# NeuroDiffGym/neurodiffeq

Hardware: AMD Instinct MI355X
Metric: collocation-points/sec (residual+bwd), 2D Laplace 65k pts, 1/2/4/8 GPU (higher is better)
Workload: dtype f32; 1 GPU; C2: Solver2D 2D Laplace, DirichletBVP2D, FCNN(2-32-32-1, tanh), Generator2D 256x256 = 65536 noisy-grid points per GPU per step, Adam(1e-3), run_train_epoch() with n_batches_train=1, n_batches_valid=0; points_per_gpu=65536, global_batch=65536, parallelism=dp1 (shard-by-batch, one all-reduce of [P+1] fp32 per step), allreduce=none (single process), inputs=pre-sampled in the reference's RNG order, resident in HBM

## Files before the change

### neurodiffeq_amd/_build.py

```python
import os

from . import _hipcc

HERE = os.path.dirname(os.path.abspath(__file__))
CSRC = os.path.join(HERE, "csrc")
LIB = os.path.join(HERE, "libndq.so")
SOURCES = [os.path.join(CSRC, "ndq_api.hip")]
HEADERS = [os.path.join(CSRC, h) for h in ("ndq_mlp.h", "ndq_tail.h", "ndq_launch.h", "ndq_wide.h", "ndq_deep.h", "ndq_sample.h", "ndq_oneshot.h")] + \
    [os.path.join(HERE, "..", "include", "ndq.h"), os.path.join(HERE, "_hipcc.py")]
LIB64 = os.path.join(HERE, "libndq64.so")
SOURCES64 = [os.path.join(CSRC, "ndq_api64.hip")]
FLAGS = []
_EXTRA = os.environ.get("NDQ_LIB_FLAGS", "").split()
if _EXTRA:
    import hashlib
    LIB = os.path.join(HERE, "libndq_" + hashlib.sha1(" ".join(_EXTRA).encode()).hexdigest()[:8] + ".so")
    FLAGS = FLAGS + _EXTRA


def is_stale():
    if not os.path.exists(LIB):
        return True
    t = os.path.getmtime(LIB)
    return any(os.path.exists(p) and os.path.getmtime(p) > t for p in SOURCES + HEADERS)


def build_lib(force=False, verbose=False):
    if not force and not is_stale():
        return LIB
    _hipcc.compile_shared(SOURCES, LIB, FLAGS, verbose=verbose)
    return LIB


def is_stale64():
    if not os.path.exists(LIB64):
        return True
    t = os.path.getmtime(LIB64)
    return any(os.path.exists(p) and os.path.getmtime(p) > t for p in SOURCES64 + HEADERS)


def build_lib64(force=False, verbose=False):
    if not force and not is_stale64():
        return LIB64
    _hipcc.compile_shared(SOURCES64, LIB64, [], verbose=verbose)
    return LIB64


if __name__ == "__main__":
    print(build_lib(force=True, verbose=True))
```

### neurodiffeq_amd/_lib.py

```python
import ctypes
import os

from . import _build

NDQ_ACT_TANH, NDQ_ACT_SIN, NDQ_ACT_SIGMOID, NDQ_ACT_SWISH, NDQ_ACT_APTX = 0, 1, 2, 3, 4
NDQ_ACT_ELU, NDQ_ACT_SOFTPLUS, NDQ_ACT_GELU = 5, 6, 7


class MlpDesc(ctypes.Structure):
    _fields_ = [("d", ctypes.c_int), ("first", ctypes.c_int), ("mask2", ctypes.c_int), ("hidden", ctypes.c_int),
                ("layers", ctypes.c_int), ("act", ctypes.c_int), ("n_out", ctypes.c_int), ("lap", ctypes.c_int),
                ("skip", ctypes.c_int), ("mask3", ctypes.c_int), ("actp", ctypes.c_int), ("widths", ctypes.c_int), ("mono", ctypes.c_int),
                ("mask4", ctypes.c_int)]

    def key(self):
        return (self.d, self.first, self.mask2, self.hidden, self.layers, self.act, self.n_out, self.lap, self.skip,
                self.mask3, self.actp, self.widths, self.mono, self.mask4)


NDQ_SAMPLE_UNIFORM, NDQ_SAMPLE_GRID, NDQ_SAMPLE_SPHERICAL = 0, 1, 2


class SamplerDesc(ctypes.Structure):
    _fields_ = [("kind", ctypes.c_int), ("d", ctypes.c_int), ("n", ctypes.c_int * 3), ("lo", ctypes.c_float * 3),
# ... 53 lines not shown
                ("lr", ctypes.c_float), ("beta1", ctypes.c_float), ("beta2", ctypes.c_float), ("eps", ctypes.c_float),
                ("weight_decay", ctypes.c_float),
                ("loss_hist", ctypes.c_void_p), ("best_loss", ctypes.c_void_p), ("best_flat", ctypes.c_void_p),
                ("allreduce", ctypes.c_void_p), ("comm", ctypes.c_void_p),
                ("next_sampler", ctypes.c_void_p), ("next_seed", ctypes.c_ulonglong), ("next_draw", ctypes.c_ulonglong),
                ("next_stream", ctypes.c_uint), ("next_coords", ctypes.c_void_p), ("next_ldc", ctypes.c_int)]


class FusedFit(ctypes.Structure):
    _fields_ = [("launch", ctypes.c_void_p), ("n_nets", ctypes.c_int), ("net", FusedStep * 4),
                ("valid_coords", ctypes.c_void_p), ("valid_n", ctypes.c_int), ("valid_ldc", ctypes.c_int),
                ("valid_blocks", ctypes.c_int), ("valid_scale", ctypes.c_float),
                ("valid_loss_partials", ctypes.c_void_p), ("valid_hist", ctypes.c_void_p), ("track_best", ctypes.c_int),
                ("pull_ok", ctypes.c_int), ("alt_params", ctypes.c_void_p * 4), ("alt_m", ctypes.c_void_p * 4),
                ("alt_v", ctypes.c_void_p * 4), ("alt_partials", ctypes.c_void_p * 4),
                ("alt_loss_partials", ctypes.c_void_p), ("alt_valid_loss_partials", ctypes.c_void_p),
                ("launch_loop", ctypes.c_void_p), ("loop_ok", ctypes.c_int)]


class NdqError(RuntimeError):
    pass


_LIB = None


def lib():
    global _LIB
    if _LIB is not None:
        return _LIB
    path = _build.LIB
    if _build.is_stale():
        try:
            _build.build_lib()
        except Exception as e:
            if not os.path.exists(path):
                raise NdqError(f"libndq.so is missing and could not be built: {e}") from e
    L = ctypes.CDLL(path)
    vp, ci, cf = ctypes.c_void_p, ctypes.c_int, ctypes.c_float
    dp = ctypes.POINTER(MlpDesc)
    L.ndq_mlp_supported.argtypes = [dp]
    L.ndq_mlp_num_streams.argtypes = [dp]
    L.ndq_mlp_num_params.argtypes = [dp]
    L.ndq_mlp_bwd_blocks.argtypes = [dp, ci]
    L.ndq_mlp_jet_fwd.argtypes = [dp, vp, ci, ci, vp, vp, ci, vp]
    L.ndq_mlp_jet_bwd.argtypes = [dp, vp, ci, ci, vp, vp, ci, vp, vp]
    L.ndq_reduce_partials.argtypes = [vp, ci, ci, vp, ci, cf, vp]
    L.ndq_adam_step.argtypes = [vp, vp, vp, vp, ci, cf, cf, cf, cf, cf, ci, vp]
    L.ndq_reduce_grad_loss.argtypes = [vp, ci, ci, vp, ci, vp, ci, vp, cf, vp]
    L.ndq_epoch_tail.argtypes = [vp, vp, vp, vp, ci, cf, cf, cf, cf, cf, ci, vp, ci, vp, ci, vp, ci, vp, ci, vp]
    L.ndq_fused_step_run.argtypes = [ctypes.POINTER(FusedStep), vp, ci, ci, ci, vp]
    L.ndq_fused_multi_step_run.argtypes = [ctypes.POINTER(FusedStep), ci, vp, vp, ci, ci, ci, vp]
    L.ndq_fused_fit_run.argtypes = [ctypes.POINTER(FusedFit), ci, vp, ci, ci, ci, ci, vp]
    L.ndq_mlp_register.argtypes = [vp]
    L.ndq_sample.argtypes = [ctypes.POINTER(SamplerDesc), ctypes.c_ulonglong, ctypes.c_ulonglong, ctypes.c_uint, vp, ci, vp]
    L.ndq_sample_table.argtypes = [ctypes.POINTER(TableSamplerDesc), ctypes.c_ulonglong, ctypes.c_ulonglong, ctypes.c_uint, vp, ci,
                                   vp]
    L.ndq_sample_plan.argtypes = [ctypes.POINTER(PlanSamplerDesc), ctypes.c_ulonglong, ctypes.c_ulonglong, ctypes.c_uint, vp, ci, vp]
    L.ndq_sample_plan_indexed.argtypes = [ctypes.POINTER(PlanSamplerDesc), ctypes.POINTER(PlanIndexDesc), ctypes.c_ulonglong,
                                          ctypes.c_ulonglong, ctypes.c_uint, vp, ci, vp]
    L.ndq_oneshot_create.argtypes = [ci, ci, ci, ctypes.POINTER(vp), ctypes.c_char_p]
    L.ndq_oneshot_connect.argtypes = [vp, ctypes.c_char_p]
    L.ndq_oneshot_allreduce.argtypes = [vp, vp, ctypes.c_size_t, ci, ci, vp, vp]
    L.ndq_oneshot_status.argtypes = [vp]
    L.ndq_oneshot_destroy.argtypes = [vp]
    for name in ("ndq_mlp_supported", "ndq_mlp_num_streams", "ndq_mlp_num_params", "ndq_mlp_bwd_blocks",
                 "ndq_mlp_jet_fwd", "ndq_mlp_jet_bwd", "ndq_reduce_partials", "ndq_adam_step", "ndq_reduce_grad_loss",
                 "ndq_epoch_tail", "ndq_fused_step_run", "ndq_sample", "ndq_sample_table", "ndq_sample_plan", "ndq_sample_plan_indexed", "ndq_mlp_register",
                 "ndq_fused_multi_step_run", "ndq_fused_fit_run", "ndq_oneshot_create", "ndq_oneshot_connect",
                 "ndq_oneshot_allreduce", "ndq_oneshot_status",
                 "ndq_oneshot_destroy"):
        getattr(L, name).restype = ci
    _LIB = L
    return L


_LIB64 = None


def lib64():
    global _LIB64
    if _LIB64 is not None:
        return _LIB64
    if _build.is_stale64():
        try:
            _build.build_lib64()
        except Exception as e:
            if not os.path.exists(_build.LIB64):
                raise NdqError(f"libndq64.so is missing and could not be built: {e}") from e
    L = ctypes.CDLL(_build.LIB64)
    vp, ci = ctypes.c_void_p, ctypes.c_int
    dp = ctypes.POINTER(MlpDesc)
    L.ndq64_mlp_supported.argtypes = [dp]
    L.ndq64_mlp_num_streams.argtypes = [dp]
    L.ndq64_mlp_num_params.argtypes = [dp]
    L.ndq64_mlp_bwd_blocks.argtypes = [dp, ci]
    L.ndq64_mlp_jet_fwd.argtypes = [dp, vp, ci, ci, vp, vp, ci, vp]
    L.ndq64_mlp_jet_bwd.argtypes = [dp, vp, ci, ci, vp, vp, ci, vp, vp]
    L.ndq64_reduce_partials.argtypes = [vp, ci, ci, vp, ci, ctypes.c_double, vp]
    L.ndq64_mlp_register.argtypes = [vp]
    cd = ctypes.c_double
    L.ndq64_adam_step.argtypes = [vp, vp, vp, vp, ci, cd, cd, cd, cd, cd, ci, vp]
    L.ndq64_epoch_tail.argtypes = [vp, vp, vp, vp, ci, cd, cd, cd, cd, cd, ci, vp, ci, vp, ci, vp, ci, vp, ci, vp]
    for name in EXPORTS64:
        getattr(L, name).restype = ci
    _LIB64 = L
    return L


EXPORTS64 = ("ndq64_mlp_register", "ndq64_mlp_supported", "ndq64_mlp_num_streams", "ndq64_mlp_num_params",
             "ndq64_mlp_bwd_blocks", "ndq64_mlp_jet_fwd", "ndq64_mlp_jet_bwd", "ndq64_reduce_partials", "ndq64_adam_step",
             "ndq64_epoch_tail")

EXPORTS = ("ndq_mlp_supported", "ndq_mlp_num_streams", "ndq_mlp_num_params", "ndq_mlp_bwd_blocks", "ndq_mlp_jet_fwd",
           "ndq_mlp_jet_bwd", "ndq_reduce_partials", "ndq_adam_step", "ndq_reduce_grad_loss", "ndq_epoch_tail",
           "ndq_fused_step_run", "ndq_sample", "ndq_sample_table", "ndq_sample_plan", "ndq_sample_plan_indexed", "ndq_mlp_register",
           "ndq_fused_multi_step_run", "ndq_fused_fit_run", "ndq_oneshot_create", "ndq_oneshot_connect", "ndq_oneshot_allreduce", "ndq_oneshot_status",
           "ndq_oneshot_destroy")


def check(rc, what):
    if rc != 0:
        raise NdqError(f"{what} failed with code {rc}" + (" (no kernel for this descriptor)" if rc == -1 else ""))
```

### neurodiffeq_amd/csrc/ndq_api.hip

```cpp
#include <cstdlib>
#include <vector>
#include "ndq_launch.h"
#include "ndq_sample.h"
#include "ndq_oneshot.h"
#include "ndq_tail.h"

extern "C" int ndq_oneshot_allreduce(const void* send, void* recv, size_t count, int dtype, int op, void* comm, void* stream);

namespace ndq {

#ifndef NDQ_CFG_TABLE
#define NDQ_CFG_TABLE(X)      \
  X(1, 0, 0, 2, 2, ACT_SIN, 1, 0)   \
  X(1, 1, 0, 2, 2, ACT_SIN, 1, 0)   \
  X(1, 1, 1, 2, 2, ACT_SIN, 1, 0)   \
  X(1, 0, 0, 2, 2, ACT_TANH, 1, 0)  \
  X(1, 1, 0, 2, 2, ACT_TANH, 1, 0)  \
  X(1, 1, 1, 2, 2, ACT_TANH, 1, 0)  \
  X(2, 0, 0, 2, 2, ACT_TANH, 1, 0)  \
  X(2, 1, 0, 2, 2, ACT_TANH, 1, 0)  \
  X(2, 1, 1, 2, 2, ACT_TANH, 1, 0)  \
  X(2, 1, 5, 2, 2, ACT_TANH, 1, 0)  \
  X(2, 1, 7, 2, 2, ACT_TANH, 1, 0)  \
  X(2, 0, 0, 4, 3, ACT_TANH, 1, 0)  \
  X(2, 1, 0, 4, 3, ACT_TANH, 1, 0)  \
  X(2, 1, 1, 4, 3, ACT_TANH, 1, 0)  \
  X(2, 1, 5, 4, 3, ACT_TANH, 1, 0)  \
  X(1, 0, 0, 2, 2, ACT_TANH, 25, 0) \
  X(1, 1, 1, 2, 2, ACT_TANH, 25, 0) \
  X(2, 1, 5, 2, 2, ACT_TANH, 3, 0)  \
  X(2, 1, 5, 2, 2, ACT_TANH, 1, 1)  \
  X(2, 1, 5, 4, 3, ACT_TANH, 1, 1)  \
  X(3, 0, 0, 2, 2, ACT_TANH, 1, 0)  \
  X(3, 1, 0, 2, 2, ACT_TANH, 1, 0)  \
  X(3, 1, 1, 2, 2, ACT_TANH, 1, 0)  \
  X(3, 1, 41, 2, 2, ACT_TANH, 1, 0) \
  X(3, 1, 41, 2, 2, ACT_TANH, 1, 1) \
  X(3, 1, 63, 2, 2, ACT_TANH, 1, 0)  \
  X(1, 0, 0, 2, 2, ACT_SIGMOID, 1, 0) \
  X(1, 1, 0, 2, 2, ACT_SIGMOID, 1, 0) \
  X(1, 1, 1, 2, 2, ACT_SIGMOID, 1, 0) \
  X(2, 0, 0, 2, 2, ACT_SIGMOID, 1, 0) \
  X(2, 1, 0, 2, 2, ACT_SIGMOID, 1, 0) \
  X(2, 1, 1, 2, 2, ACT_SIGMOID, 1, 0) \
  X(2, 1, 5, 2, 2, ACT_SIGMOID, 1, 0) \
  X(2, 1, 7, 2, 2, ACT_SIGMOID, 1, 0) \
  X(2, 1, 5, 2, 2, ACT_SIGMOID, 1, 1) \
  X(1, 0, 0, 2, 2, ACT_SWISH, 1, 0) \
  X(1, 1, 0, 2, 2, ACT_SWISH, 1, 0) \
  X(1, 1, 1, 2, 2, ACT_SWISH, 1, 0) \
  X(2, 0, 0, 2, 2, ACT_SWISH, 1, 0) \
  X(2, 1, 0, 2, 2, ACT_SWISH, 1, 0) \
  X(2, 1, 1, 2, 2, ACT_SWISH, 1, 0) \
  X(2, 1, 5, 2, 2, ACT_SWISH, 1, 0) \
  X(2, 1, 7, 2, 2, ACT_SWISH, 1, 0) \
  X(2, 1, 5, 2, 2, ACT_SWISH, 1, 1)
#endif

// ... 566 lines not shown
        const ndq_fused_step& s = f->net[k];
        ndq::PullNet& n = pa.net[k];
        n.part = c.PART[in][k];
        n.p_in = c.P[in][k]; n.m_in = c.M[in][k]; n.v_in = c.V[in][k];
        n.p_out = c.P[out][k]; n.m_out = c.M[out][k]; n.v_out = c.V[out][k];
        n.grad = s.grad; n.best_flat = track ? s.best_flat : nullptr; n.len = s.n_params;
        n.adam = adam_consts(s.lr, s.beta1, s.beta2, s.eps, s.weight_decay, w.adam_step);
      }
      parity ^= 1;
    }
    const bool train_part = e < c.n_epochs, valid_part = c.valid && e >= 1;
    if (train_part && !c.train_coords[e]) return NDQ_EINVAL;
    int rc = f->launch(train_part ? c.train_coords[e] : nullptr, s0.ldc, train_part ? s0.n : 0, c.P[e & 1],
                       train_part ? c.PART[e & 1] : nullptr, c.LP[e & 1], s0.seed, valid_part ? f->valid_coords : nullptr,
                       f->valid_ldc, valid_part ? f->valid_n : 0, c.VP[e & 1], &pa, c.stream);
    if (rc) return rc;
  }
  return fit_closing_tail(c, last & 1, parity);
}

static int fit_loop(const FitCall& c, long long stride, int parity) {
  const ndq_fused_fit* f = c.f;
  const ndq_fused_step& s0 = f->net[0];
  const int last = fit_last_launch(c);
  int in = 0;
  for (int e0 = 0; e0 <= last; e0 += ndq::kLoopMaxLaunches, in ^= 1) {
    const int e1 = e0 + ndq::kLoopMaxLaunches <= last + 1 ? e0 + ndq::kLoopMaxLaunches : last + 1;
    const int out = in ^ 1;
    ndq::LoopArgs L{};
    L.e0 = e0; L.e1 = e1; L.n_epochs = c.n_epochs; L.has_valid = c.valid ? 1 : 0; L.track_best = f->track_best;
    L.hist_index = c.hist_index; L.valid_index = c.valid_index; L.parity = parity; L.coord_stride = stride;
    L.lp_in = c.LP[in]; L.vp_in = c.VP[in]; L.lp_out = c.LP[out]; L.vp_out = c.VP[out];
    L.lscale = s0.seed; L.vscale = f->valid_scale;
    L.loss_hist = s0.loss_hist; L.loss_slot = s0.loss_slot; L.valid_hist = f->valid_hist; L.best_loss = s0.best_loss;
    for (int k = 0; k < f->n_nets; ++k) {
      const ndq_fused_step& s = f->net[k];
      ndq::LoopNet& n = L.net[k];
      n.p_in = c.P[in][k]; n.m_in = c.M[in][k]; n.v_in = c.V[in][k]; n.part_in = c.PART[in][k];
      n.p_out = c.P[out][k]; n.m_out = c.M[out][k]; n.v_out = c.V[out][k]; n.part_out = c.PART[out][k];
      n.grad = s.grad; n.best_flat = s.best_flat;
      n.lr = s.lr; n.b1 = s.beta1; n.b2 = s.beta2; n.eps = s.eps; n.wd = s.weight_decay;
      for (int e = e0 > 1 ? e0 : 1; e < e1; ++e) {
        const ndq::AdamConsts a = adam_consts(s.lr, s.beta1, s.beta2, s.eps, s.weight_decay, launch_finishes(c, e).adam_step);
        n.bc1[e - e0] = a.bc1; n.bc2s[e - e0] = a.bc2s;
      }
    }
    int rc = f->launch_loop(c.train_coords[0], s0.ldc, s0.n, s0.seed, c.valid ? f->valid_coords : nullptr, f->valid_ldc,
                            c.valid ? f->valid_n : 0, &L, c.stream);
    if (rc) return rc;
  }
  return fit_closing_tail(c, in, parity ^ (last & 1));
}

extern "C" {

int ndq_fused_fit_run(const ndq_fused_fit* f, int n_epochs, const float* const* train_coords, int adam_step,
                      int hist_index, int valid_index, int parity, void* stream) {
  if (!f || !f->launch || f->n_nets < 1 || f->n_nets > 4 || n_epochs < 0 || (n_epochs > 0 && (!train_coords || adam_step <= 0)) ||
      hist_index < 0 || valid_index < 0 || (parity != 0 && parity != 1) || f->track_best < 0 || f->track_best > 2)
    return NDQ_EINVAL;
  const ndq_fused_step& s0 = f->net[0];
  const bool valid = f->valid_coords != nullptr;
  if (!valid && n_epochs == 0) return NDQ_EINVAL;
  if (!s0.best_loss || (n_epochs > 0 && (!s0.loss_hist || !s0.loss_partials || s0.n <= 0 || s0.blocks <= 0))) return NDQ_EINVAL;
  if (valid && (!f->valid_loss_partials || !f->valid_hist || f->valid_n <= 0 || f->valid_blocks <= 0)) return NDQ_EINVAL;
  if (f->track_best == 2 && !valid) return NDQ_EINVAL;
  FitCall c{f, n_epochs, train_coords, adam_step, hist_index, valid_index, stream, valid};
  c.max_lparts = s0.blocks > f->valid_blocks ? s0.blocks : f->valid_blocks;
  c.LP[0] = s0.loss_partials; c.LP[1] = f->alt_loss_partials;
  c.VP[0] = f->valid_loss_partials; c.VP[1] = f->alt_valid_loss_partials;
  bool pull = f->pull_ok != 0 && n_epochs >= 2 && s0.blocks * f->n_nets <= ndq::kPullMaxWork && f->alt_loss_partials &&
              (!valid || f->alt_valid_loss_partials);
  for (int k = 0; k < f->n_nets; ++k) {
    const ndq_fused_step& s = f->net[k];
    if (!s.params || s.n_params <= 0 || (f->track_best && !s.best_flat)) return NDQ_EINVAL;
    if (n_epochs > 0 && (!s.partials || !s.grad || !s.adam_m || !s.adam_v || !s.loss_slot)) return NDQ_EINVAL;
    if (s.n_params > c.max_params) c.max_params = s.n_params;
    c.P[0][k] = s.params; c.M[0][k] = s.adam_m; c.V[0][k] = s.adam_v; c.PART[0][k] = s.partials;
    c.P[1][k] = f->alt_params[k]; c.M[1][k] = f->alt_m[k]; c.V[1][k] = f->alt_v[k]; c.PART[1][k] = f->alt_partials[k];
    pull = pull && c.P[1][k] && c.M[1][k] && c.V[1][k] && c.PART[1][k];
  }
  if (!pull) return fit_two_launch(c, parity);
  bool loop = f->loop_ok != 0 && f->launch_loop && s0.blocks == 1 && (!valid || f->valid_blocks == 1) &&
              f->n_nets <= ndq::kLoopMaxNets;
  long long stride = 0;
  if (loop) {
    if (!train_coords[0] || !train_coords[1]) return NDQ_EINVAL;
    stride = train_coords[1] - train_coords[0];
    for (int e = 2; e < n_epochs && loop; ++e) {
      if (!train_coords[e]) return NDQ_EINVAL;
      loop = train_coords[e] - train_coords[0] == stride * e;
    }
  }
  return loop ? fit_loop(c, stride, parity) : fit_pull(c, parity);
}

int ndq_adam_step(float* params, const float* grad, float* exp_avg, float* exp_avg_sq, int len, float lr, float beta1,
                  float beta2, float eps, float weight_decay, int step, void* stream) {
  if (!params || !grad || !exp_avg || !exp_avg_sq || len <= 0 || step <= 0) return NDQ_EINVAL;
  hipLaunchKernelGGL(adam_kernel<float>, dim3((len + 255) / 256), dim3(256), 0, static_cast<hipStream_t>(stream), params, grad,
                     exp_avg, exp_avg_sq, len, adam_consts(lr, beta1, beta2, eps, weight_decay, step));
  return (int)hipGetLastError();
}

int ndq_sample(const ndq_sampler_desc* desc, unsigned long long seed, unsigned long long draw, unsigned stream_id,
               float* coords, int ldc, void* stream) {
  return ndq::launch_sample(desc, seed, draw, stream_id, coords, ldc, (hipStream_t)stream);
}

int ndq_sample_table(const ndq_table_sampler_desc* desc, unsigned long long seed, unsigned long long draw,
                     unsigned stream_id, float* coords, int ldc, void* stream) {
  return ndq::launch_sample_table(desc, seed, draw, stream_id, coords, ldc, (hipStream_t)stream);
}

int ndq_sample_plan(const ndq_plan_sampler_desc* desc, unsigned long long seed, unsigned long long draw,
                    unsigned stream_id, float* coords, int ldc, void* stream) {
  return ndq::launch_sample_plan(desc, seed, draw, stream_id, coords, ldc, (hipStream_t)stream);
}

int ndq_sample_plan_indexed(const ndq_plan_sampler_desc* desc, const ndq_plan_index_desc* index, unsigned long long seed,
                            unsigned long long draw, unsigned stream_id, float* coords, int ldc, void* stream) {
  return ndq::launch_sample_plan_indexed(desc, index, seed, draw, stream_id, coords, ldc, (hipStream_t)stream);
}

}

extern "C" {

int ndq_oneshot_create(int rank, int world, int max_len, void** out, unsigned char* handle64) {
  if (!out || !handle64 || world < 1 || world > ndq::kOneshotMaxRanks || rank < 0 || rank >= world || max_len < 1)
    return NDQ_EINVAL;
  ndq::Oneshot* c = new (std::nothrow) ndq::Oneshot();
  if (!c) return NDQ_EINVAL;
  std::memset(c, 0, sizeof(*c));
// ... 71 lines not shown
```

### neurodiffeq_amd/engine.py

```python
import ctypes
import functools
import os

import torch

from . import _lib, codegen, generators
from .networks import FlatParams, describe
from .symbolic import Graph, Sym, TraceUnsupported, trace_scope

_c_vp = ctypes.c_void_p


def _ptr(t):
    return _c_vp(t.data_ptr())


_raw_stream = getattr(torch._C, "_cuda_getCurrentRawStream", None) or \
    (lambda idx: torch.cuda.current_stream(idx).cuda_stream)


def _round_up(n, m):
    return (n + m - 1) // m * m


class _Lib64:

    def __init__(self):
        self._lib = _lib.lib64()

    def __getattr__(self, name):
        return getattr(self._lib, name.replace("ndq_", "ndq64_", 1))


def _ends(c):
    n = c.numel()
    if n == 0:
        return ()
    if c.is_contiguous():
        p, e = c.data_ptr(), c.element_size()
        return (ctypes.string_at(p, e), ctypes.string_at(p + (n - 1) * e, e))
    f = c.detach().reshape(-1)
    return (f[0].item(), f[-1].item())


class library_code:
    __slots__ = ("ctx",)

    def __enter__(self):
        self.ctx = torch._C.DisableTorchFunction() if torch._C._len_torch_function_stack() else None
        if self.ctx is not None:
            self.ctx.__enter__()
        return self

    def __exit__(self, *exc):
        if self.ctx is not None:
            self.ctx.__exit__(*exc)
            self.ctx = None
        return False

    def user_code(self):
        return _UserCode(self)


class _UserCode:
    __slots__ = ("lc", "was")

    def __init__(self, lc):
        self.lc = lc

    def __enter__(self):
        self.was = self.lc.ctx is not None
# ... 871 lines not shown

    def fast_train_epoch(self, batch, optimizer, adam_slot, track_best, n_global=None, dist=None):
        fs = self.fast_state()
        b, n = self.upload(batch)
        fp = self.flat[0]
        fp.sync()
        m, v, group, step = adam_slot
        key = (n, b["ld"], id(b))
        st = fs["structs"].get(key)
        if st is None:
            st = _lib.FusedStep()
            st.launch = b["fused_launch"]
            self._fill_step(st, 0, n, b["ld"], b["fused_blocks"], b["fused_partials"], b["fused_loss_partials"])
            fs["structs"][key] = st
        n_global = n if n_global is None else n_global
        st.params = fp.flat.data_ptr()
        st.seed = 1.0 / (float(n_global) * self.loss_norm)
        st.best_flat = fs["best_flat"][0].data_ptr() if track_best else None
        self._set_adam(st, m, v, group)
        stream = self._stream()
        coords = self._coord_ptr(b, 0)
        hist_index, parity = fs["pending"], fs["parity"]
        src = generators.device_source(batch) if dist is None else None
        if src is not None and src.prefetch and b["coords_rows"] is not None:
            st.next_sampler = ctypes.addressof(src.desc)
            st.next_seed, st.next_draw, st.next_stream = src.seed, src.draw, src.stream_id
            nxt = src.block_of(src.draw)
            st.next_coords, st.next_ldc = nxt.data_ptr(), nxt.shape[1]
        else:
            src, st.next_sampler = None, None
        direct = dist.direct(self.device, fp.numel + 1) if dist is not None else None
        if dist is None or direct is not None:
            st.allreduce, st.comm = direct if direct is not None else (None, None)
            rc = self.L.ndq_fused_step_run(ctypes.byref(st), coords, step, hist_index, parity, stream)
            _lib.check(rc, "ndq_fused_step_run")
            if src is not None:
                src.prefetched = src.draw
        else:
            st.adam_m = st.adam_v = None
            st.allreduce = st.comm = None
            rc = self.L.ndq_fused_step_run(ctypes.byref(st), coords, step, hist_index, parity, stream)
            _lib.check(rc, "ndq_fused_step_run")
            dist.all_reduce_flat(fp.grad_loss)
            rc = self.L.ndq_epoch_tail(*self._tail_args(fp, adam_slot), _c_vp(st.loss_slot), 1, _ptr(fs["loss_hist"]),
                                       hist_index, _ptr(fs["best_loss"]), parity,
                                       _ptr(fs["best_flat"][0]) if track_best else None, 1, stream)
            _lib.check(rc, "ndq_epoch_tail")
        fs["pending"] += 1
        fs["parity"] ^= 1

    FIT_RUN = os.environ.get("NDQ_FIT_RUN", "1") != "0"
    FIT_PULL = os.environ.get("NDQ_FIT_PULL", "1") != "0"
    FIT_LOOP = os.environ.get("NDQ_FIT_LOOP", "1") != "0"

    def fit_ready(self):
        return self.FIT_RUN and self.fusedk is not None and not self.f64 and not self.n_theta

    def resident_ptr(self, batch):
        if batch[0].device.type != "cuda" or len(batch) != self.n_coords:
            return None
        ld = self._resident_ld(batch)
        return (batch[0].data_ptr(), ld) if ld else None

    def stage_batches(self, host_block, n, reserve=0):
        K = host_block.shape[0]
        ld = _round_up(n, 64)
        st = self.__dict__.setdefault("_stage", dict(pinned=[None, None], events=[None, None], next=0, dev=[None, None]))
        i = st["next"]
        st["next"] ^= 1
        need = K * self.n_coords * ld
        if st["pinned"][i] is None or st["pinned"][i].numel() < need:
            if st["events"][i] is not None:
                st["events"][i].synchronize()
            size = max(need, reserve * self.n_coords * ld)
            for j in (0, 1):
                if st["pinned"][j] is None or st["pinned"][j].numel() < size:
                    if st["events"][j] is not None:
                        st["events"][j].synchronize()
                    st["pinned"][j] = torch.zeros(size, dtype=torch.float32, device="cpu", pin_memory=True)
                    st["dev"][j] = torch.zeros(size, dtype=torch.float32, device=self.device)
        elif st["events"][i] is not None:
            st["events"][i].synchronize()
        pinned = st["pinned"][i][:need].view(K, self.n_coords, ld)
        import numpy as np
        np.copyto(pinned.numpy()[:, :, :n], host_block.detach().numpy(), casting="same_kind")
        dev = st["dev"][i][:need].view(K, self.n_coords, ld)
        dev.copy_(pinned, non_blocking=True)
        ev = st["events"][i] or torch.cuda.Event()
        ev.record()
        st["events"][i] = ev
        return dev, ld

    def fit_run(self, train_ptrs, n, ld, adam_slots, valid=None, track_best=0, n_global=None):
        fs = self.fast_state()
        K = len(train_ptrs)
        if K:
            self._fit_last_n = n
        fk = self.fused_variant(n if K else (getattr(self, "_fit_last_n", None) or valid[1]))
        key = (id(fk), n if K else 0, ld if K else 0, (valid[1], valid[2]) if valid else None)
        cache = fs.setdefault("fit", {})
        ent = cache.get(key)
        if ent is None:
            if len(cache) >= 8:
                cache.pop(next(iter(cache)))
            dev, f32 = self.device, torch.float32
            ff = _lib.FusedFit()
            ff.launch = ctypes.cast(fk.lib.ndq_fused_launch_tv, ctypes.c_void_p).value
            ff.n_nets = len(self.flat)
            keep = []
            blocks = fk.blocks(n) if K else 0
            lparts = torch.zeros(max(blocks, 1), dtype=f32, device=dev)
            keep.append(lparts)
            for k, fp in enumerate(self.flat):
                part = torch.empty(blocks, fp.numel, dtype=f32, device=dev) if K else None
                keep.append(part)
                self._fill_step(ff.net[k], k, *((n, ld, blocks) if K else (0, 0, 0)), part, lparts)
                ff.net[k].best_flat = fs["best_flat"][k].data_ptr()
            if valid is not None:
                vparts = torch.zeros(fk.blocks(valid[1]), dtype=f32, device=dev)
                keep.append(vparts)
                ff.valid_n, ff.valid_ldc, ff.valid_blocks = valid[1], valid[2], vparts.numel()
                ff.valid_scale = 1.0 / (float(valid[1]) * self.loss_norm)
                ff.valid_loss_partials, ff.valid_hist = vparts.data_ptr(), fs["valid_hist"].data_ptr()
            ff.pull_ok = 0
            if K and self.FIT_PULL and 0 < blocks * len(self.flat) <= 16 and fk.lib.ndq_fused_pull_ok():
                ff.pull_ok = 1
                for k, fp in enumerate(self.flat):
                    alt = [torch.zeros(fp.numel, dtype=f32, device=dev) for _ in range(3)]
                    apart = torch.empty(blocks, fp.numel, dtype=f32, device=dev)
                    keep.extend(alt + [apart])
                    ff.alt_params[k], ff.alt_m[k], ff.alt_v[k] = (t.data_ptr() for t in alt)
                    ff.alt_partials[k] = apart.data_ptr()
                alp = torch.zeros(max(blocks, 1), dtype=f32, device=dev)
                keep.append(alp)
                ff.alt_loss_partials = alp.data_ptr()
                if valid is not None:
                    avp = torch.zeros(ff.valid_blocks, dtype=f32, device=dev)
                    keep.append(avp)
                    ff.alt_valid_loss_partials = avp.data_ptr()
                if self.FIT_LOOP and blocks == 1 and (valid is None or ff.valid_blocks == 1) and len(self.flat) <= 2 \
                        and fk.lib.ndq_fused_loop_ok():
                    ff.launch_loop = ctypes.cast(fk.lib.ndq_fused_launch_loop, ctypes.c_void_p).value
                    ff.loop_ok = 1
            ent = cache[key] = (ff, keep, fk, {}, (_c_vp * 1)(), ctypes.byref(ff))
        ff = ent[0]
        step0 = 1
        last = ent[3]
        for k, fp in enumerate(self.flat):
            fp.sync()
            if K:
                m, v, group, step0 = adam_slots[k]
                now = (fp.flat.data_ptr(), n if n_global is None else n_global, m.data_ptr(), v.data_ptr(), group["lr"],
                       group["betas"], group["eps"], group["weight_decay"])
            else:
                now = (fp.flat.data_ptr(),)
            if last.get(k) != now:
                last[k] = now
                st = ff.net[k]
                st.params = now[0]
                if K:
                    st.seed = 1.0 / (float(now[1]) * self.loss_norm)
                    self._set_adam(st, m, v, group)
        vc = valid[0] if valid is not None else None
        if last.get("v") != (vc, track_best):
            last["v"] = (vc, track_best)
            ff.valid_coords = vc
            ff.track_best = track_best
        if K == 1:
            coords = ent[4]
            coords[0] = train_ptrs[0]
        else:
            coords = (_c_vp * max(K, 1))(*train_ptrs) if K else None
        rc = self.L.ndq_fused_fit_run(ent[5], K, coords, step0, fs["pending"], fs["pending_valid"], fs["parity"],
                                      self._stream())
        _lib.check(rc, "ndq_fused_fit_run")
        tails = K + (1 if valid is not None else 0)
        fs["pending"] += K
        if valid is not None:
            fs["pending_valid"] += max(K, 1)
        fs["parity"] ^= tails & 1

    def fast_flush(self):
        fs = getattr(self, "_fast", None)
        if fs is None or (fs["pending"] == 0 and fs["pending_valid"] == 0):
            return [], [], None
        k, kv = fs["pending"], fs["pending_valid"]
        vals = torch.cat([fs["loss_hist"][:k], fs["valid_hist"][:kv],
                          fs["best_loss"][fs["parity"]:fs["parity"] + 1]]).tolist()
        fs["pending"] = fs["pending_valid"] = 0
        return vals[:k], vals[k:k + kv], vals[k + kv]

    def step(self, batch, train, slot=0, accumulate=False, n_global=None, lo=0, hi=None, want_funcs=False,
             want_resid=False):
        b, n = self.upload(batch, lo, hi)
        n_global = n if n_global is None else n_global
        stream = self._stream()
        self.set_batch_size(n_global)
        self.refresh_theta()
        if train and not accumulate and not self.verify_fused(b, n, n_global):
            b, n = self.upload(batch, lo, hi)
        if b["fusedk"] is not None:
            self.fused_closure(b, n, stream, train, n_global, slot, accumulate, want_funcs, want_resid)
            return b, n
        self.forward(b, n, stream)
        seed = self.pointwise(b, n, stream, train, n_global, want_funcs, want_resid)
        if train:
            self.backward(b, n, stream, accumulate, after_forward=True)
            self.reduce_theta(b, b["pw_blocks"], stream, accumulate)
        self.reduce_loss(b, stream, seed, slot)
        return b, n
```

### neurodiffeq_amd/solvers.py

```python
import inspect
import sys
import warnings
from abc import ABC, abstractmethod
from copy import deepcopy
from itertools import chain

import torch
import torch.nn as nn

from . import _lib
from .conditions import BaseCondition
from .generators import (Generator1D, Generator2D, GeneratorSpherical, SamplerGenerator, draws_are_static,
                         draws_have_fixed_size, device_source, on_default_device)
from . import autograd_ops
from .losses import _losses
from .networks import FCNN, describe
from .neurodiffeq import safe_diff as diff
from .optim import FusedAdam
from .symbolic import MetricTraceUnsupported, TraceUnsupported, captured_unchanged
from .networks import STRUCTURE as _net_structure
import os as _os
_QUICK_KEY = _os.environ.get("NDQ_QUICK_KEY", "1") != "0"
_LC = []

# ... 623 lines not shown
            pass
        elif train and nb == 1 and len(system.flat) > 1 and system.fast_ready(shard) and len({s[3] for s in slots}) == 1:
            system.fast_train_epoch_multi(first_batch, slots, track_best)
        elif train and nb == 1 and len(system.flat) == 1 and system.fast_ready(shard):
            batch = first_batch
            n_all = batch[0].shape[0]
            if shard is not None:
                lo, hi = shard.bounds(n_all)
                if (lo, hi) != (0, n_all):
                    batch = [c[lo:hi] for c in batch]
            system.fast_train_epoch(batch, self.optimizer, slots[0], track_best,
                                    n_global=shard.global_n(n_all) if shard else n_all, dist=shard)
        else:
            if system.loss_buf.numel() < nb:
                system.loss_buf = torch.zeros(nb, dtype=system.dt, device=self.device)
            batches = [first_batch]
            if nb > 1:
                with self._lc.user_code():
                    batches += [self._generate_batch(key) for _ in range(nb - 1)]
            if not train and nb > 1:
                if all(b is batches[0] for b in batches[1:]) and batches[0][0].device.type != "cuda":
                    batches = batches[:1]
                else:
                    k0 = system.static_key(batches[0])
                    if k0 is not None and all(system.static_key(b) == k0 for b in batches[1:]):
                        batches = batches[:1]
            for batch_id, batch in enumerate(batches):
                n_all = batch[0].shape[0]
                lo, hi = shard.bounds(n_all) if shard else (0, n_all)
                system.step(batch, train=train, slot=batch_id, accumulate=(batch_id > 0),
                            n_global=shard.global_n(n_all) if shard else n_all, lo=lo, hi=hi)
            if shard:
                shard.all_reduce(system, len(batches), train=train)
            system.epoch_tail(key, len(batches), track_best, slots)
        if train:
            for fp in system.flat:
                if not fp.grads_attached():
                    fp.attach_grads()
        self._phase = key
        return True

    def _fit_epoch(self, key, system, batch, slots):
        train = key == "train"
        if train:
            if len({s[3] for s in slots}) != 1:
                return False
            src = device_source(batch)
            if src is not None and src.prefetch:
                return False
        n_all = batch[0].shape[0]
        if system.needs_check(n_all):
            return False
        b, n = system.upload(batch)
        ptr = system._coord_ptr(b, 0).value
        if train:
            system.fit_run([ptr], n, b["ld"], slots, None, track_best=1 if self.n_batches["valid"] == 0 else 0)
        else:
            system.fit_run([], 0, 0, None, (ptr, n, b["ld"]), track_best=2)
        return True

    _PER_EPOCH_METHODS = ("run_train_epoch", "run_valid_epoch", "_run_epoch", "_generate_batch", "_generate_train_batch",
                          "_generate_valid_batch")

    FIT_CHUNK = 256

    def _fit_chunk(self, remaining):
        system = self._fused_sys
        if system is None or self.dist is not None or self.n_batches["train"] != 1 or remaining < 2:
            return 0
        if not self._native_ok() or not system.fit_ready() or getattr(system.program, "loss_probe", None) is not None:
            return 0
        if system.n_data:
            return 0
        cls = type(self)
        if any(getattr(cls, m) is not getattr(BaseSolver, m) for m in self._PER_EPOCH_METHODS):
            return 0
        nv = self.n_batches["valid"]
        tg, vg = self.generator["train"], self.generator["valid"]
        if not draws_have_fixed_size(tg) or (nv > 0 and not draws_are_static(vg)):
            return 0
        if type(tg.generator).__name__ == "DeviceGenerator":
            return 0
        if self._fused_system(system.n_coords) is not system:
            return 0
        if self._eq_watch_blocks_chunks():
            return 0
        if not self._equations_unchanged(system, force=True):
            self._fused_key = None
            return 0
        n = tg.size
        if system.needs_check(n):
            return 0
        if not all(self.optimizer.bound(fp) for fp in system.flat):
            return 0
        if len({self.optimizer._steps.get(id(fp)) for fp in system.flat}) != 1:
            return 0
        fs = system.fast_state()
        if max(fs["pending"], fs["pending_valid"]) + 2 > system.HIST:
            self._flush_device_history()
        k_max = min(self.FIT_CHUNK, max(2, (64 << 20) // (4 * system.n_coords * (n + 63))))
        K = min(remaining, k_max, system.HIST - max(fs["pending"], fs["pending_valid"]))
        if K < 2:
            return 0
        if fs["pending"] == 0 and fs["pending_valid"] == 0:
            fs["best_loss"].fill_(float("inf") if self._lowest_loss is None else float(self._lowest_loss))
        valid = None
        if nv > 0:
# ... 520 lines not shown
```

Baseline: 3.311 billion collocation-points/s.

## Add persistent native fit plan to cut per-epoch host launch overhead

Adds a native fit-plan object that caches the fused-fit descriptor, counters and a ring of batch coordinate pointers, so a single-batch train epoch becomes one ctypes call. Epochs no longer rebuild the FusedFit struct, re-validate every field, or marshal a coordinate array each step. Python only pushes deltas such as optimizer params, seed, counters or stream when they change. The plan path always takes the two-launch route and bypasses the pull/loop variants, which could cost device-side efficiency, and it adds state-consistency risk between the Python and native counters.

```diff
diff --git a/neurodiffeq_amd/_build.py b/neurodiffeq_amd/_build.py
--- a/neurodiffeq_amd/_build.py
+++ b/neurodiffeq_amd/_build.py
@@ -6,7 +6,7 @@
 CSRC = os.path.join(HERE, "csrc")
 LIB = os.path.join(HERE, "libndq.so")
 SOURCES = [os.path.join(CSRC, "ndq_api.hip")]
-HEADERS = [os.path.join(CSRC, h) for h in ("ndq_mlp.h", "ndq_tail.h", "ndq_launch.h", "ndq_wide.h", "ndq_deep.h", "ndq_sample.h", "ndq_oneshot.h")] + \
+HEADERS = [os.path.join(CSRC, h) for h in ("ndq_mlp.h", "ndq_tail.h", "ndq_launch.h", "ndq_wide.h", "ndq_deep.h", "ndq_sample.h", "ndq_oneshot.h", "ndq_fit_plan.h")] + \
     [os.path.join(HERE, "..", "include", "ndq.h"), os.path.join(HERE, "_hipcc.py")]
 LIB64 = os.path.join(HERE, "libndq64.so")
 SOURCES64 = [os.path.join(CSRC, "ndq_api64.hip")]
diff --git a/neurodiffeq_amd/_lib.py b/neurodiffeq_amd/_lib.py
--- a/neurodiffeq_amd/_lib.py
+++ b/neurodiffeq_amd/_lib.py
@@ -129,6 +129,20 @@
     L.ndq_fused_step_run.argtypes = [ctypes.POINTER(FusedStep), vp, ci, ci, ci, vp]
     L.ndq_fused_multi_step_run.argtypes = [ctypes.POINTER(FusedStep), ci, vp, vp, ci, ci, ci, vp]
     L.ndq_fused_fit_run.argtypes = [ctypes.POINTER(FusedFit), ci, vp, ci, ci, ci, ci, vp]
+    L.ndq_fit_plan_create.argtypes = [ctypes.POINTER(FusedFit), ci, ci, ci, vp, ctypes.POINTER(vp)]
+    L.ndq_fit_plan_destroy.argtypes = [vp]
+    L.ndq_fit_plan_destroy.restype = None
+    L.ndq_fit_plan_set_net.argtypes = [vp, ci, vp, vp, vp, cf, cf, cf, cf, cf]
+    L.ndq_fit_plan_set_seed.argtypes = [vp, cf]
+    L.ndq_fit_plan_set_track_best.argtypes = [vp, ci]
+    L.ndq_fit_plan_set_stream.argtypes = [vp, vp]
+    L.ndq_fit_plan_set_counters.argtypes = [vp, ci, ci, ci]
+    L.ndq_fit_plan_get_counters.argtypes = [vp, ctypes.POINTER(ci), ctypes.POINTER(ci), ctypes.POINTER(ci)]
+    L.ndq_fit_plan_set_batch.argtypes = [vp, ci, vp, ci, ci]
+    L.ndq_fit_plan_epoch.argtypes = [vp, ci]
+    for name in FIT_PLAN_EXPORTS:
+        if name != "ndq_fit_plan_destroy":
+            getattr(L, name).restype = ci
     L.ndq_mlp_register.argtypes = [vp]
     L.ndq_sample.argtypes = [ctypes.POINTER(SamplerDesc), ctypes.c_ulonglong, ctypes.c_ulonglong, ctypes.c_uint, vp, ci, vp]
     L.ndq_sample_table.argtypes = [ctypes.POINTER(TableSamplerDesc), ctypes.c_ulonglong, ctypes.c_ulonglong, ctypes.c_uint, vp, ci,
@@ -189,6 +203,10 @@
              "ndq64_mlp_bwd_blocks", "ndq64_mlp_jet_fwd", "ndq64_mlp_jet_bwd", "ndq64_reduce_partials", "ndq64_adam_step",
              "ndq64_epoch_tail")
 
+FIT_PLAN_EXPORTS = ("ndq_fit_plan_create", "ndq_fit_plan_destroy", "ndq_fit_plan_set_net", "ndq_fit_plan_set_seed",
+                    "ndq_fit_plan_set_track_best", "ndq_fit_plan_set_stream", "ndq_fit_plan_set_counters",
+                    "ndq_fit_plan_get_counters", "ndq_fit_plan_set_batch", "ndq_fit_plan_epoch")
+
 EXPORTS = ("ndq_mlp_supported", "ndq_mlp_num_streams", "ndq_mlp_num_params", "ndq_mlp_bwd_blocks", "ndq_mlp_jet_fwd",
            "ndq_mlp_jet_bwd", "ndq_reduce_partials", "ndq_adam_step", "ndq_reduce_grad_loss", "ndq_epoch_tail",
            "ndq_fused_step_run", "ndq_sample", "ndq_sample_table", "ndq_sample_plan", "ndq_sample_plan_indexed", "ndq_mlp_register",
diff --git a/neurodiffeq_amd/csrc/ndq_api.hip b/neurodiffeq_amd/csrc/ndq_api.hip
--- a/neurodiffeq_amd/csrc/ndq_api.hip
+++ b/neurodiffeq_amd/csrc/ndq_api.hip
@@ -4,6 +4,7 @@
 #include "ndq_sample.h"
 #include "ndq_oneshot.h"
 #include "ndq_tail.h"
+#include "ndq_fit_plan.h"
 
 extern "C" int ndq_oneshot_allreduce(const void* send, void* recv, size_t count, int dtype, int op, void* comm, void* stream);
 
@@ -676,34 +677,40 @@
   return fit_closing_tail(c, in, parity ^ (last & 1));
 }
 
-extern "C" {
-
-int ndq_fused_fit_run(const ndq_fused_fit* f, int n_epochs, const float* const* train_coords, int adam_step,
-                      int hist_index, int valid_index, int parity, void* stream) {
-  if (!f || !f->launch || f->n_nets < 1 || f->n_nets > 4 || n_epochs < 0 || (n_epochs > 0 && (!train_coords || adam_step <= 0)) ||
-      hist_index < 0 || valid_index < 0 || (parity != 0 && parity != 1) || f->track_best < 0 || f->track_best > 2)
-    return NDQ_EINVAL;
+static void fit_call_fill(FitCall& c) {
+  const ndq_fused_fit* f = c.f;
   const ndq_fused_step& s0 = f->net[0];
-  const bool valid = f->valid_coords != nullptr;
-  if (!valid && n_epochs == 0) return NDQ_EINVAL;
-  if (!s0.best_loss || (n_epochs > 0 && (!s0.loss_hist || !s0.loss_partials || s0.n <= 0 || s0.blocks <= 0))) return NDQ_EINVAL;
-  if (valid && (!f->valid_loss_partials || !f->valid_hist || f->valid_n <= 0 || f->valid_blocks <= 0)) return NDQ_EINVAL;
-  if (f->track_best == 2 && !valid) return NDQ_EINVAL;
-  FitCall c{f, n_epochs, train_coords, adam_step, hist_index, valid_index, stream, valid};
+  c.max_params = 0;
   c.max_lparts = s0.blocks > f->valid_blocks ? s0.blocks : f->valid_blocks;
   c.LP[0] = s0.loss_partials; c.LP[1] = f->alt_loss_partials;
   c.VP[0] = f->valid_loss_partials; c.VP[1] = f->alt_valid_loss_partials;
-  bool pull = f->pull_ok != 0 && n_epochs >= 2 && s0.blocks * f->n_nets <= ndq::kPullMaxWork && f->alt_loss_partials &&
-              (!valid || f->alt_valid_loss_partials);
   for (int k = 0; k < f->n_nets; ++k) {
     const ndq_fused_step& s = f->net[k];
-    if (!s.params || s.n_params <= 0 || (f->track_best && !s.best_flat)) return NDQ_EINVAL;
-    if (n_epochs > 0 && (!s.partials || !s.grad || !s.adam_m || !s.adam_v || !s.loss_slot)) return NDQ_EINVAL;
     if (s.n_params > c.max_params) c.max_params = s.n_params;
     c.P[0][k] = s.params; c.M[0][k] = s.adam_m; c.V[0][k] = s.adam_v; c.PART[0][k] = s.partials;
     c.P[1][k] = f->alt_params[k]; c.M[1][k] = f->alt_m[k]; c.V[1][k] = f->alt_v[k]; c.PART[1][k] = f->alt_partials[k];
-    pull = pull && c.P[1][k] && c.M[1][k] && c.V[1][k] && c.PART[1][k];
-  }
+  }
+}
+
+static int ndq_fit_plan_enqueue(const ndq_fit_plan& p, const float* const* coords) {
+  FitCall c{&p.f, 1, coords, p.adam_step, p.hist_index, p.valid_index, p.stream, false};
+  fit_call_fill(c);
+  return fit_two_launch(c, p.parity);
+}
+
+extern "C" {
+
+int ndq_fused_fit_run(const ndq_fused_fit* f, int n_epochs, const float* const* train_coords, int adam_step,
+                      int hist_index, int valid_index, int parity, void* stream) {
+  const int bad = ndq::fit_validate(f, n_epochs, train_coords != nullptr, adam_step, hist_index, valid_index, parity);
+  if (bad) return bad;
+  const ndq_fused_step& s0 = f->net[0];
+  const bool valid = f->valid_coords != nullptr;
+  FitCall c{f, n_epochs, train_coords, adam_step, hist_index, valid_index, stream, valid};
+  fit_call_fill(c);
+  bool pull = f->pull_ok != 0 && n_epochs >= 2 && s0.blocks * f->n_nets <= ndq::kPullMaxWork && f->alt_loss_partials &&
+              (!valid || f->alt_valid_loss_partials);
+  for (int k = 0; k < f->n_nets; ++k) pull = pull && c.P[1][k] && c.M[1][k] && c.V[1][k] && c.PART[1][k];
   if (!pull) return fit_two_launch(c, parity);
   bool loop = f->loop_ok != 0 && f->launch_loop && s0.blocks == 1 && (!valid || f->valid_blocks == 1) &&
               f->n_nets <= ndq::kLoopMaxNets;
diff --git a/neurodiffeq_amd/csrc/ndq_fit_plan.h b/neurodiffeq_amd/csrc/ndq_fit_plan.h
--- /dev/null
+++ b/neurodiffeq_amd/csrc/ndq_fit_plan.h
@@ -0,0 +1,137 @@
+#pragma once
+#include <new>
+#include "../../include/ndq.h"
+
+namespace ndq {
+
+inline int fit_validate(const ndq_fused_fit* f, int n_epochs, bool has_coords, int adam_step, int hist_index, int valid_index,
+                        int parity) {
+  if (!f || !f->launch || f->n_nets < 1 || f->n_nets > 4 || n_epochs < 0 || (n_epochs > 0 && (!has_coords || adam_step <= 0)) ||
+      hist_index < 0 || valid_index < 0 || (parity != 0 && parity != 1) || f->track_best < 0 || f->track_best > 2)
+    return NDQ_EINVAL;
+  const ndq_fused_step& s0 = f->net[0];
+  const bool valid = f->valid_coords != nullptr;
+  if (!valid && n_epochs == 0) return NDQ_EINVAL;
+  if (!s0.best_loss || (n_epochs > 0 && (!s0.loss_hist || !s0.loss_partials || s0.n <= 0 || s0.blocks <= 0))) return NDQ_EINVAL;
+  if (valid && (!f->valid_loss_partials || !f->valid_hist || f->valid_n <= 0 || f->valid_blocks <= 0)) return NDQ_EINVAL;
+  if (f->track_best == 2 && !valid) return NDQ_EINVAL;
+  for (int k = 0; k < f->n_nets; ++k) {
+    const ndq_fused_step& s = f->net[k];
+    if (!s.params || s.n_params <= 0 || (f->track_best && !s.best_flat)) return NDQ_EINVAL;
+    if (n_epochs > 0 && (!s.partials || !s.grad || !s.adam_m || !s.adam_v || !s.loss_slot)) return NDQ_EINVAL;
+  }
+  return 0;
+}
+
+constexpr int kFitPlanSlots = 16;
+
+}
+
+struct ndq_fit_plan;
+extern "C" {
+int ndq_fit_plan_create(const ndq_fused_fit* f, int adam_step, int hist_index, int parity, void* stream, ndq_fit_plan** out);
+void ndq_fit_plan_destroy(ndq_fit_plan* plan);
+int ndq_fit_plan_set_net(ndq_fit_plan* plan, int k, float* params, float* adam_m, float* adam_v, float lr, float beta1,
+                         float beta2, float eps, float weight_decay);
+int ndq_fit_plan_set_seed(ndq_fit_plan* plan, float seed);
+int ndq_fit_plan_set_track_best(ndq_fit_plan* plan, int track_best);
+int ndq_fit_plan_set_stream(ndq_fit_plan* plan, void* stream);
+int ndq_fit_plan_set_counters(ndq_fit_plan* plan, int adam_step, int hist_index, int parity);
+int ndq_fit_plan_get_counters(const ndq_fit_plan* plan, int* adam_step, int* hist_index, int* parity);
+int ndq_fit_plan_set_batch(ndq_fit_plan* plan, int slot, const float* coords, int n, int ldc);
+int ndq_fit_plan_epoch(ndq_fit_plan* plan, int batch_slot);
+}
+
+struct ndq_fit_plan {
+  ndq_fused_fit f;
+  void* stream;
+  int adam_step, hist_index, valid_index, parity;
+  const float* ring[ndq::kFitPlanSlots];
+};
+
+static int ndq_fit_plan_enqueue(const ndq_fit_plan& p, const float* const* coords);
+
+namespace ndq {
+inline int fit_plan_check(const ndq_fit_plan& p) {
+  if (p.f.valid_coords) return NDQ_EINVAL;
+  return fit_validate(&p.f, 1, true, p.adam_step, p.hist_index, p.valid_index, p.parity);
+}
+template <class Edit>
+inline int fit_plan_update(ndq_fit_plan* p, Edit edit) {
+  if (!p) return NDQ_EINVAL;
+  ndq_fit_plan q = *p;
+  edit(q);
+  const int rc = fit_plan_check(q);
+  if (rc == 0) *p = q;
+  return rc;
+}
+}
+
+extern "C" {
+
+int ndq_fit_plan_create(const ndq_fused_fit* f, int adam_step, int hist_index, int parity, void* stream, ndq_fit_plan** out) {
+  if (!f || !out) return NDQ_EINVAL;
+  ndq_fit_plan q{};
+  q.f = *f;
+  q.stream = stream;
+  q.adam_step = adam_step; q.hist_index = hist_index; q.valid_index = 0; q.parity = parity;
+  const int rc = ndq::fit_plan_check(q);
+  if (rc) return rc;
+  ndq_fit_plan* p = new (std::nothrow) ndq_fit_plan(q);
+  if (!p) return NDQ_EINVAL;
+  *out = p;
+  return 0;
+}
+
+void ndq_fit_plan_destroy(ndq_fit_plan* p) { delete p; }
+
+int ndq_fit_plan_set_net(ndq_fit_plan* p, int k, float* params, float* adam_m, float* adam_v, float lr, float beta1,
+                         float beta2, float eps, float weight_decay) {
+  if (!p || k < 0 || k >= p->f.n_nets) return NDQ_EINVAL;
+  return ndq::fit_plan_update(p, [&](ndq_fit_plan& q) {
+    ndq_fused_step& s = q.f.net[k];
+    s.params = params; s.adam_m = adam_m; s.adam_v = adam_v;
+    s.lr = lr; s.beta1 = beta1; s.beta2 = beta2; s.eps = eps; s.weight_decay = weight_decay;
+  });
+}
+
+int ndq_fit_plan_set_seed(ndq_fit_plan* p, float seed) {
+  return ndq::fit_plan_update(p, [&](ndq_fit_plan& q) { q.f.net[0].seed = seed; });
+}
+
+int ndq_fit_plan_set_track_best(ndq_fit_plan* p, int track_best) {
+  return ndq::fit_plan_update(p, [&](ndq_fit_plan& q) { q.f.track_best = track_best; });
+}
+
+int ndq_fit_plan_set_stream(ndq_fit_plan* p, void* stream) {
+  return ndq::fit_plan_update(p, [&](ndq_fit_plan& q) { q.stream = stream; });
+}
+
+int ndq_fit_plan_set_counters(ndq_fit_plan* p, int adam_step, int hist_index, int parity) {
+  return ndq::fit_plan_update(p, [&](ndq_fit_plan& q) { q.adam_step = adam_step; q.hist_index = hist_index; q.parity = parity; });
+}
+
+int ndq_fit_plan_get_counters(const ndq_fit_plan* p, int* adam_step, int* hist_index, int* parity) {
+  if (!p || !adam_step || !hist_index || !parity) return NDQ_EINVAL;
+  *adam_step = p->adam_step; *hist_index = p->hist_index; *parity = p->parity;
+  return 0;
+}
+
+int ndq_fit_plan_set_batch(ndq_fit_plan* p, int slot, const float* coords, int n, int ldc) {
+  if (!p || slot < 0 || slot >= ndq::kFitPlanSlots || !coords) return NDQ_EINVAL;
+  if (n != p->f.net[0].n || ldc != p->f.net[0].ldc) return NDQ_EINVAL;
+  p->ring[slot] = coords;
+  return 0;
+}
+
+int ndq_fit_plan_epoch(ndq_fit_plan* p, int batch_slot) {
+  if (!p || batch_slot < 0 || batch_slot >= ndq::kFitPlanSlots || !p->ring[batch_slot]) return NDQ_EINVAL;
+  const int rc = ndq_fit_plan_enqueue(*p, &p->ring[batch_slot]);
+  if (rc) return rc;
+  p->adam_step += 1;
+  p->hist_index += 1;
+  p->parity ^= 1;
+  return 0;
+}
+
+}
diff --git a/neurodiffeq_amd/engine.py b/neurodiffeq_amd/engine.py
--- a/neurodiffeq_amd/engine.py
+++ b/neurodiffeq_amd/engine.py
@@ -17,6 +17,24 @@
 
 _raw_stream = getattr(torch._C, "_cuda_getCurrentRawStream", None) or \
     (lambda idx: torch.cuda.current_stream(idx).cuda_stream)
+
+
+class _FitPlan:
+    __slots__ = ("L", "h", "epoch", "n", "ld", "fk", "nets", "seed_n", "track_best", "stream", "step", "hist", "parity",
+                 "slots", "ring", "next", "keep")
+
+    def __init__(self, L, ff, n, ld, fk, step, hist, parity, stream):
+        h = _c_vp()
+        _lib.check(L.ndq_fit_plan_create(ctypes.byref(ff), step, hist, parity, _c_vp(stream), ctypes.byref(h)), "ndq_fit_plan_create")
+        self.L, self.h, self.epoch = L, h, L.ndq_fit_plan_epoch
+        self.n, self.ld, self.fk = n, ld, fk
+        self.step, self.hist, self.parity, self.stream = step, hist, parity, stream
+        self.slots, self.ring, self.next = {}, [], 0
+
+    def __del__(self):
+        h, self.h = self.h, None
+        if h:
+            self.L.ndq_fit_plan_destroy(h)
 
 
 def _round_up(n, m):
@@ -994,6 +1012,8 @@
     FIT_RUN = os.environ.get("NDQ_FIT_RUN", "1") != "0"
     FIT_PULL = os.environ.get("NDQ_FIT_PULL", "1") != "0"
     FIT_LOOP = os.environ.get("NDQ_FIT_LOOP", "1") != "0"
+    FIT_PLAN = os.environ.get("NDQ_FIT_PLAN", "1") != "0"
+    FIT_PLAN_RING = 16
 
     def fit_ready(self):
         return self.FIT_RUN and self.fusedk is not None and not self.f64 and not self.n_theta
@@ -1036,6 +1056,12 @@
     def fit_run(self, train_ptrs, n, ld, adam_slots, valid=None, track_best=0, n_global=None):
         fs = self.fast_state()
         K = len(train_ptrs)
+        plan_route = K == 1 and valid is None and self.FIT_PLAN
+        if plan_route:
+            pl = fs.get("plan")
+            if pl is not None and pl.n == n and pl.ld == ld and pl.fk is self.fused_variant(n):
+                self._fit_last_n = n
+                return self._plan_epoch(fs, pl, train_ptrs[0], adam_slots, track_best, n if n_global is None else n_global)
         if K:
             self._fit_last_n = n
         fk = self.fused_variant(n if K else (getattr(self, "_fit_last_n", None) or valid[1]))
@@ -1108,6 +1134,15 @@
             last["v"] = (vc, track_best)
             ff.valid_coords = vc
             ff.track_best = track_best
+        if plan_route:
+            stream = _raw_stream(self._dev_index)
+            pl = _FitPlan(self.L, ff, n, ld, fk, step0, fs["pending"], fs["parity"], stream)
+            pl.nets = [[fp.flat, s[0], s[1], s[2], s[2]["lr"], s[2]["betas"], s[2]["eps"], s[2]["weight_decay"]]
+                       for fp, s in zip(self.flat, adam_slots)]
+            pl.seed_n, pl.track_best = n if n_global is None else n_global, track_best
+            pl.keep = ent
+            fs["plan"] = pl
+            return self._plan_epoch(fs, pl, train_ptrs[0], adam_slots, track_best, pl.seed_n, synced=True)
         if K == 1:
             coords = ent[4]
             coords[0] = train_ptrs[0]
@@ -1121,6 +1156,56 @@
         if valid is not None:
             fs["pending_valid"] += max(K, 1)
         fs["parity"] ^= tails & 1
+
+    def _plan_epoch(self, fs, pl, ptr, adam_slots, track_best, seed_n, synced=False):
+        L = pl.L
+        step0 = adam_slots[0][3]
+        if not synced:
+            k = 0
+            for fp in self.flat:
+                fp.sync()
+                m, v, group, _ = adam_slots[k]
+                c = pl.nets[k]
+                if not (fp.flat is c[0] and m is c[1] and v is c[2] and group is c[3] and group["lr"] == c[4]
+                        and group["betas"] == c[5] and group["eps"] == c[6] and group["weight_decay"] == c[7]):
+                    b1, b2 = group["betas"]
+                    _lib.check(L.ndq_fit_plan_set_net(pl.h, k, fp.flat.data_ptr(), m.data_ptr(), v.data_ptr(), group["lr"], b1, b2,
+                                                      group["eps"], group["weight_decay"]), "ndq_fit_plan_set_net")
+                    pl.nets[k] = [fp.flat, m, v, group, group["lr"], group["betas"], group["eps"], group["weight_decay"]]
+                k += 1
+            if pl.seed_n != seed_n:
+                _lib.check(L.ndq_fit_plan_set_seed(pl.h, 1.0 / (float(seed_n) * self.loss_norm)), "ndq_fit_plan_set_seed")
+                pl.seed_n = seed_n
+            if pl.track_best != track_best:
+                _lib.check(L.ndq_fit_plan_set_track_best(pl.h, track_best), "ndq_fit_plan_set_track_best")
+                pl.track_best = track_best
+            hist, parity = fs["pending"], fs["parity"]
+            if pl.step != step0 or pl.hist != hist or pl.parity != parity:
+                _lib.check(L.ndq_fit_plan_set_counters(pl.h, step0, hist, parity), "ndq_fit_plan_set_counters")
+                pl.step, pl.hist, pl.parity = step0, hist, parity
+            stream = _raw_stream(self._dev_index)
+            if stream != pl.stream:
+                _lib.check(L.ndq_fit_plan_set_stream(pl.h, stream), "ndq_fit_plan_set_stream")
+                pl.stream = stream
+        slot = pl.slots.get(ptr)
+        if slot is None:
+            ring = pl.ring
+            if len(ring) < min(self.FIT_PLAN_RING, 16):
+                slot = len(ring)
+                ring.append(ptr)
+            else:
+                slot = pl.next % len(ring)
+                pl.next = slot + 1
+                pl.slots.pop(ring[slot], None)
+                ring[slot] = ptr
+            _lib.check(L.ndq_fit_plan_set_batch(pl.h, slot, ptr, pl.n, pl.ld), "ndq_fit_plan_set_batch")
+            pl.slots[ptr] = slot
+        rc = pl.epoch(pl.h, slot)
+        if rc:
+            _lib.check(rc, "ndq_fit_plan_epoch")
+        pl.step = step0 + 1
+        pl.hist = fs["pending"] = pl.hist + 1
+        pl.parity = fs["parity"] = pl.parity ^ 1
 
     def fast_flush(self):
         fs = getattr(self, "_fast", None)
diff --git a/neurodiffeq_amd/solvers.py b/neurodiffeq_amd/solvers.py
--- a/neurodiffeq_amd/solvers.py
+++ b/neurodiffeq_amd/solvers.py
@@ -699,7 +699,8 @@
         if system.needs_check(n_all):
             return False
         b, n = system.upload(batch)
-        ptr = system._coord_ptr(b, 0).value
+        rows = b["coords_rows"]
+        ptr = (rows[0] if rows is not None else b["coords_own"][0]).data_ptr()
         if train:
             system.fit_run([ptr], n, b["ld"], slots, None, track_best=1 if self.n_batches["valid"] == 0 else 0)
         else:
```

Measured after the change: 3.295 billion collocation-points/s. No clear change (-0.5%).
